# facebookresearch/detectron2

Measured on NVIDIA H100. Metric: Mask R-CNN R50-FPN training hot-path images/sec (custom-op path fwd+bwd, 2 images/GPU), higher is better.
Workload: dtype f32

## Files before the change

detectron2_b200/csrc/deform_conv_tc.cu:

```cuda
#include <algorithm>
#include <cstdlib>

#include "common.cuh"
#include "tc_common.cuh"

using namespace d2b_tc;

namespace {

constexpr int kWorkerWarps = 16;
constexpr int kWorkers = kWorkerWarps * 32;
constexpr int kThreads = kWorkers + 128;
constexpr int kLaunchRegs = (65536 / kThreads) & ~7;
constexpr int kWorkerRegs = 112, kSideRegs = 24;
static_assert(kWorkers * kWorkerRegs + (kThreads - kWorkers) * kSideRegs <= kThreads * kLaunchRegs,
              "register budget exceeds the launch allocation");
constexpr int kMaxBN = 128;
constexpr int kRowsPerHalf = 128 / (2 * kWorkerWarps);
constexpr int kTile = 16384;
constexpr int kMaxSmem = 227 * 1024;
constexpr int kGcolPitch = 132;

struct TC {
  int N, Cin, H, W, Cout, kh, kw, sh, sw, ph, pw, dh, dw, G, DG, Ho, Wo, cpg, opg, cpdg, KK, HoWo;
  int pack, SG, cps, ops, cbs, U;
  int tiles_img;
  int stages_img;
  int MC;
  int nks;
  long long off_bs, mask_bs;
  int mask_sigmoid;
};

struct Epi {
  const float* scale;
  const float* shift;
  int relu;
};

struct K1P { int BN, noct, goct, nkp, ksplit, S, tap_bytes, stage_bytes, red; };
struct K2P { int mper, msplit, tap_bytes; };
struct K3P { int BN, noct, sper, nsplit, S, stage_bytes; };

inline size_t align256(size_t v) { return (v + 255) & ~(size_t)255; }

bool make_tc(const d2b_dcn_params* p, TC& d) {
  if (!p) return false;
  d.N = p->N; d.Cin = p->Cin; d.H = p->H; d.W = p->W; d.Cout = p->Cout; d.kh = p->kh; d.kw = p->kw;
// ... 172 lines not shown
  const float* __restrict__ p = xcb + (uint32_t)(code >> 4) * Cin;
  const float4 z = make_float4(0.f, 0.f, 0.f, 0.f);
  t.v0 = (code & 1) ? __ldg(reinterpret_cast<const float4*>(p)) : z;
  t.v1 = (code & 2) ? __ldg(reinterpret_cast<const float4*>(p + Cin)) : z;
  t.v2 = (code & 4) ? __ldg(reinterpret_cast<const float4*>(p + rs)) : z;
  t.v3 = (code & 8) ? __ldg(reinterpret_cast<const float4*>(p + (rs + Cin))) : z;
}

__device__ __forceinline__ void interp4(const Taps4& t, float w0, float w1, float w2, float w3, float (&v)[4]) {
  const F2 z = f2_pack(0.f, 0.f), p0 = f2_pack(w0, w0), p1 = f2_pack(w1, w1), p2 = f2_pack(w2, w2), p3 = f2_pack(w3, w3);
  F2 a = f2_fma(p0, f2_pack(t.v0.x, t.v0.y), z), b = f2_fma(p0, f2_pack(t.v0.z, t.v0.w), z);
  a = f2_fma(p1, f2_pack(t.v1.x, t.v1.y), a);
  b = f2_fma(p1, f2_pack(t.v1.z, t.v1.w), b);
  a = f2_fma(p2, f2_pack(t.v2.x, t.v2.y), a);
  b = f2_fma(p2, f2_pack(t.v2.z, t.v2.w), b);
  a = f2_fma(p3, f2_pack(t.v3.x, t.v3.y), a);
  b = f2_fma(p3, f2_pack(t.v3.z, t.v3.w), b);
  f2_unpack(a, v[0], v[1]);
  f2_unpack(b, v[2], v[3]);
}

__device__ __forceinline__ void gather_store(const Taps4& t, int4 tap, uint8_t* a_hi, uint8_t* a_lo, uint32_t off,
                                             bool split) {
  const float lh = __int_as_float(tap.y), lw = __int_as_float(tap.z), m = __int_as_float(tap.w);
  const float hh = 1.f - lh, hw = 1.f - lw;
  float v[4];
  interp4(t, hh * hw * m, hh * lw * m, lh * hw * m, lh * lw * m, v);
  uint2 hi, lo;
  split4(v, hi, lo);
  *reinterpret_cast<uint2*>(a_hi + off) = hi;
  if (split) *reinterpret_cast<uint2*>(a_lo + off) = lo;
}

template <int BN, int kTransA, int kSplit>
__device__ __forceinline__ void mma_stage_(float (&acc)[BN / 4], uint32_t a_hi, uint32_t a_lo, uint32_t b_hi, uint32_t b_lo) {
  const int g = (threadIdx.x >> 7);
  const uint32_t ao = kTransA ? (uint32_t)(g & 1) * 8192u : (uint32_t)(g & 1) * 64u * 128u;
  const uint32_t bo = (uint32_t)(g >> 1) * (uint32_t)(BN / 2) * 128u;
  const uint32_t lbo = kTransA ? 8192u : 0u;
  wgmma_fence();
#pragma unroll
  for (int kk = 0; kk < 4; ++kk) {
    const uint32_t ak = ao + (kTransA ? (uint32_t)kk * 2048u : (uint32_t)kk * 32u), bk = bo + (uint32_t)kk * 32u;
    Wgmma<BN / 2, kTransA>::mma(acc, wgmma_desc(a_hi + ak, lbo, 1024), wgmma_desc(b_hi + bk, 0, 1024), 1);
    if (kSplit) {
      Wgmma<BN / 2, kTransA>::mma(acc, wgmma_desc(a_hi + ak, lbo, 1024), wgmma_desc(b_lo + bk, 0, 1024), 1);
      Wgmma<BN / 2, kTransA>::mma(acc, wgmma_desc(a_lo + ak, lbo, 1024), wgmma_desc(b_hi + bk, 0, 1024), 1);
    }
  }
  wgmma_commit();
}
template <int BN, int kTransA>
__device__ __forceinline__ void mma_stage(float (&acc)[BN / 4], uint32_t a_hi, uint32_t a_lo, uint32_t b_hi, uint32_t b_lo,
                                          int split) {
  if (split) mma_stage_<BN, kTransA, 1>(acc, a_hi, a_lo, b_hi, b_lo);
  else mma_stage_<BN, kTransA, 0>(acc, a_hi, a_lo, b_hi, b_lo);
}

template <int BN>
__device__ __forceinline__ int acc_row(int i) {
  const int t = threadIdx.x & 127;
  return (threadIdx.x >> 7 & 1) * 64 + (t >> 5) * 16 + ((t & 31) >> 2) + ((i >> 1) & 1) * 8;
}
template <int BN>
__device__ __forceinline__ int acc_col(int i) {
  return (threadIdx.x >> 8) * (BN / 2) + (i >> 2) * 8 + (threadIdx.x & 3) * 2 + (i & 1);
}

template <int BN>
__device__ __forceinline__ void fwd_epilogue(const float (&acc)[BN / 4], const Epi& ep, const TC& d, const K1P& k,
                                             float* __restrict__ out, int b, int p0, int oc0) {
  const bool add_shift = ep.shift != nullptr && blockIdx.z == 0;
#pragma unroll
  for (int i = 0; i < BN / 4; ++i) {
    const int p = p0 + acc_row<BN>(i);
    if (p >= d.HoWo) continue;
    const int oc = oc0 + acc_col<BN>(i);
    float* dst = out + ((size_t)b * d.Cout + oc) * d.HoWo + p;
    float v = acc[i];
    if (k.red) {
      red_add(dst, v + ((add_shift && !ep.scale && !ep.relu) ? __ldg(ep.shift + oc) : 0.f));
    } else {
      if (ep.scale) v *= __ldg(ep.scale + oc);
      if (ep.shift) v += __ldg(ep.shift + oc);
      if (ep.relu) v = fmaxf(v, 0.f);
      *dst = v;
    }
  }
}

template <int BN>
__global__ void __launch_bounds__(kThreads, 1) dcn_fwd_tc_kernel(const float* __restrict__ xh,
                                                                   const float* __restrict__ offset,
                                                                   const float* __restrict__ mask,
                                                                   const uint8_t* __restrict__ wt, const Epi ep, const TC d,
                                                                   const K1P k, const int split, float* __restrict__ out,
                                                                   uint8_t* __restrict__ cols) {
  extern __shared__ uint8_t smem_raw[];
  uint8_t* smem = smem_raw + ((1024u - (smem_u32(smem_raw) & 1023u)) & 1023u);
  int4* taps = reinterpret_cast<int4*>(smem + k.S * k.stage_bytes);
  uint64_t* bars = reinterpret_cast<uint64_t*>(reinterpret_cast<uint8_t*>(taps) + k.tap_bytes);
  uint64_t* full_bar = bars;
  uint64_t* empty_bar = bars + k.S;

  const int tid = threadIdx.x, warp = tid >> 5, lane = tid & 31;
  const int b = blockIdx.x / d.tiles_img, p0 = (blockIdx.x - b * d.tiles_img) * 128;
  const int sg = blockIdx.y / k.goct, oct = blockIdx.y - sg * k.goct;
  const int kp0 = blockIdx.z * k.nkp, nkp = min(d.KK, kp0 + k.nkp) - kp0;
  const int nt = nkp * d.cbs;
  const int dg0 = (sg * d.cps) / d.cpdg;
// ... 23 lines not shown
    const float* __restrict__ ximg = xh + (size_t)b * d.H * d.W * d.Cin - (size_t)(d.W + 1) * d.Cin;
    const uint32_t ucin = (uint32_t)d.Cin, urs = (uint32_t)(d.W * d.Cin);
    float acc[BN / 4];
#pragma unroll
    for (int i = 0; i < BN / 4; ++i) acc[i] = 0.f;
    int kpl = 0, cb = 0;
    auto stage = [&](int t) {
      const int s = t % k.S;
      const uint32_t par = (uint32_t)((t / k.S) & 1);
      const int cbase = sg * d.cps + cb * 64;
      const int4* __restrict__ tp = taps + ((cbase / d.cpdg - dg0) * nkp + kpl) * 128;
      const float* __restrict__ xc = ximg + cbase + q * 4;
      uint8_t* a_hi = smem + s * k.stage_bytes;
      uint8_t* a_lo = a_hi + kTile;
      mbar_wait(&empty_bar[s], par ^ 1u);
      {
        int4 tap[kRowsPerHalf];
        Taps4 c[kRowsPerHalf];
#pragma unroll
        for (int j = 0; j < kRowsPerHalf; ++j) tap[j] = tp[warp * 2 * kRowsPerHalf + j * 2 + half];
#pragma unroll
        for (int j = 0; j < kRowsPerHalf; ++j) load_corners(xc, ucin, urs, tap[j].x, c[j]);
#pragma unroll
        for (int j = 0; j < kRowsPerHalf; ++j) {
          const uint32_t r = (uint32_t)(warp * 2 * kRowsPerHalf + j * 2 + half);
          gather_store(c[j], tap[j], a_hi, a_lo, swz128(r, (uint32_t)(q >> 1)) + (uint32_t)(q & 1) * 8u, split != 0);
        }
      }
      fence_proxy_async();
      __syncwarp();
      if (lane == 0) mbar_arrive(&full_bar[s]);
      mbar_wait(&full_bar[s], par);
      const uint32_t sa = smem_u32(a_hi), sb = sa + 2 * kTile;
      mma_stage<BN, 0>(acc, sa, sa + kTile, sb, sb + (uint32_t)BN * 128u, split);
      if (++cb == d.cbs) { cb = 0; ++kpl; }
    };
    stage(0);
    for (int t = 1; t < nt; ++t) {
      stage(t);
      wgmma_wait<1>();
      __syncwarp();
      if (lane == 0) mbar_arrive(&empty_bar[(t - 1) % k.S]);
    }
    wgmma_wait<0>();
    fwd_epilogue<BN>(acc, ep, d, k, out, b, p0, sg * d.ops + oct * k.BN);
  } else if (warp == kWorkerWarps) {
    if (lane == 0) {
      const uint32_t bytes = (uint32_t)(split ? 2 : 1) * (uint32_t)k.BN * 128u;
      for (int t = 0; t < nt; ++t) {
        const int s = t % k.S;
        const uint32_t par = (uint32_t)((t / k.S) & 1);
        mbar_wait(&empty_bar[s], par ^ 1u);
        const size_t tile = ((size_t)(sg * k.noct + oct) * d.U + (size_t)kp0 * d.cbs + t);
        mbar_arrive_expect_tx(&full_bar[s], bytes);
        bulk_g2s(smem + s * k.stage_bytes + 2 * kTile, wt + tile * (size_t)(2 * k.BN * 128), bytes, &full_bar[s]);
      }
    }
  } else if (warp == kWorkerWarps + 1) {
    if (saving && lane == 0) {
      const uint32_t tile_bytes = (uint32_t)(split ? 2 : 1) * (uint32_t)kTile;
      for (int t = 0; t < nt; ++t) {
        const int s = t % k.S;
        const uint32_t par = (uint32_t)((t / k.S) & 1);
        mbar_wait(&full_bar[s], par);
        const size_t tile = ((size_t)blockIdx.x * d.SG + sg) * d.U + (size_t)kp0 * d.cbs + t;
        bulk_s2g(cols + tile * tile_bytes, smem + s * k.stage_bytes, tile_bytes);
        bulk_commit();
        bulk_wait_read0();
        mbar_arrive(&empty_bar[s]);
      }
      bulk_wait0();
    }
  }
}

template <int BN>
__global__ void __launch_bounds__(kThreads, 1) dcn_fwd_cols_kernel(const uint8_t* __restrict__ cols,
                                                                   const uint8_t* __restrict__ wt, const Epi ep, const TC d,
                                                                   const K1P k, const int split, float* __restrict__ out) {
  extern __shared__ uint8_t smem_raw[];
  uint8_t* smem = smem_raw + ((1024u - (smem_u32(smem_raw) & 1023u)) & 1023u);
  uint64_t* bars = reinterpret_cast<uint64_t*>(smem + k.S * k.stage_bytes);
  uint64_t* full_bar = bars;
  uint64_t* empty_bar = bars + k.S;

  const int tid = threadIdx.x, warp = tid >> 5, lane = tid & 31;
  const int tile = blockIdx.x / k.goct, oct = 1 + (blockIdx.x - tile * k.goct);
  const int b = tile / d.tiles_img, p0 = (tile - b * d.tiles_img) * 128;
  const int sg = blockIdx.y;
  const int kp0 = blockIdx.z * k.nkp, nkp = min(d.KK, kp0 + k.nkp) - kp0;
  const int nt = nkp * d.cbs;

  if (tid == 0) {
    for (int s = 0; s < k.S; ++s) {
      mbar_init(&full_bar[s], 1);
      mbar_init(&empty_bar[s], kWorkerWarps);
    }
    mbar_init_fence();
  }
  __syncthreads();
  if (warp < kWorkerWarps) reg_alloc<kWorkerRegs>();
  else reg_dealloc<kSideRegs>();

  if (warp < kWorkerWarps) {
    float acc[BN / 4];
#pragma unroll
    for (int i = 0; i < BN / 4; ++i) acc[i] = 0.f;
    auto issue = [&](int t) {
      const int s = t % k.S;
      mbar_wait(&full_bar[s], (uint32_t)((t / k.S) & 1));
      const uint32_t sa = smem_u32(smem + s * k.stage_bytes), sb = sa + 2 * kTile;
      mma_stage<BN, 0>(acc, sa, sa + kTile, sb, sb + (uint32_t)BN * 128u, split);
    };
    issue(0);
    for (int t = 1; t < nt; ++t) {
      issue(t);
      wgmma_wait<1>();
      __syncwarp();
      if (lane == 0) mbar_arrive(&empty_bar[(t - 1) % k.S]);
    }
    wgmma_wait<0>();
    fwd_epilogue<BN>(acc, ep, d, k, out, b, p0, sg * d.ops + oct * k.BN);
  } else if (warp == kWorkerWarps) {
    if (lane == 0) {
      const uint32_t parts = split ? 2u : 1u;
      const uint32_t abytes = parts * (uint32_t)kTile;
      const size_t u0 = (size_t)kp0 * d.cbs;
      const uint8_t* asrc = cols + (((size_t)tile * d.SG + sg) * d.U + u0) * abytes;
      const uint8_t* bsrc = wt + ((size_t)(sg * k.noct + oct) * d.U + u0) * (size_t)(2 * BN * 128);
      int s = 0;
      uint32_t par = 1u;
      for (int t = nt; t > 0; --t, asrc += abytes, bsrc += 2 * BN * 128) {
        mbar_wait(&empty_bar[s], par);
        mbar_arrive_expect_tx(&full_bar[s], abytes / 128u * (128u + BN));
        bulk_g2s(smem + s * k.stage_bytes, asrc, abytes, &full_bar[s]);
        bulk_g2s(smem + s * k.stage_bytes + 2 * kTile, bsrc, abytes / 128u * BN, &full_bar[s]);
        if (++s == k.S) {
          s = 0;
          par ^= 1u;
        }
      }
    }
  }
}

__global__ void __launch_bounds__(kThreads, 1) dcn_bwd_data_tc_kernel(const float* __restrict__ xh,
                                                                      const float* __restrict__ offset,
                                                                      const float* __restrict__ mask,
                                                                      const uint8_t* __restrict__ gt,
                                                                      const uint8_t* __restrict__ wt, const TC d,
                                                                      const K2P k, const int split,
                                                                      float* __restrict__ gxh, float* __restrict__ goff,
                                                                      float* __restrict__ gmask) {
  extern __shared__ uint8_t smem_raw[];
  uint8_t* smem = smem_raw + ((1024u - (smem_u32(smem_raw) & 1023u)) & 1023u);
  constexpr int kStage = 4 * kTile;
// ... 71 lines not shown
      float v = (b1 ? u1 : u0) + __shfl_xor_sync(0xffffffffu, b1 ? u0 : u1, 1);
      {
        const int j = q >> 2, which = q & 3;
        const int row = warp * 2 * R + j * 2 + half;
        const int p = p0 + row;
        if (which < 3 && p < d.HoWo) {
          if (which < 2) {
            if (goff) red_add(goff + (size_t)b * d.off_bs + ((size_t)cur_dg * 2 * d.KK + 2 * cur_kp + which) * d.HoWo + p, v);
          } else if (gmask) {
            if (d.mask_sigmoid) {
              const float m = __int_as_float(taps[((cur_dg - dg0) * nkp + (cur_kp - kp0)) * 128 + row].w);
              v *= m * (1.f - m);
            }
            red_add(gmask + (size_t)b * d.mask_bs + ((size_t)cur_dg * d.KK + cur_kp) * d.HoWo + p, v);
          }
        }
      }
#pragma unroll
      for (int j = 0; j < R; ++j) sh[j] = sw[j] = sm[j] = 0.f;
    };

    for (int ml = 0; ml < nm; ++ml) {
      const int buf = ml & 1;
      const int m = m0 + ml;
      const int nu = (2 * m + 1 < d.U) ? 2 : 1;
      {
        float acc[32];
#pragma unroll
        for (int i = 0; i < 32; ++i) acc[i] = 0.f;
        for (int ks = 0; ks < d.nks; ++ks) {
          const int c = ml * d.nks + ks, s = c & 1;
          mbar_wait(&full_bar[s], (uint32_t)((c >> 1) & 1));
          const uint32_t sa = smem_u32(smem + s * kStage);
          mma_stage<128, 0>(acc, sa, sa + kTile, sa + 2 * kTile, sa + 3 * kTile, split);
          wgmma_wait<0>();
          __syncwarp();
          if (lane == 0) mbar_arrive(&empty_bar[s]);
        }
#pragma unroll
        for (int i = 0; i < 32; i += 2)
          *reinterpret_cast<float2*>(gcol + acc_row<128>(i) * kGcolPitch + acc_col<128>(i)) = make_float2(acc[i], acc[i + 1]);
      }
      named_bar_sync(1, kWorkers);
      for (int ul = 0; ul < nu; ++ul) {
        const int u = 2 * m + ul;
        const int kp = u / d.cbs, cb = u - kp * d.cbs;
        const int cbase = sg * d.cps + cb * 64;
        const int dg = cbase / d.cpdg;
        if (kp != cur_kp || dg != cur_dg) {
          flush();
          cur_kp = kp;
          cur_dg = dg;
        }
        const int4* __restrict__ tp = taps + ((dg - dg0) * nkp + (kp - kp0)) * 128;
        const float* __restrict__ xc = ximg + cbase + q * 4;
        float* __restrict__ gc = gimg + cbase + q * 4;
        constexpr int kB2 = 2;
#pragma unroll
        for (int it = 0; it < R / kB2; ++it) {
          int4 tap[kB2];
          Taps4 c[kB2];
#pragma unroll
          for (int e = 0; e < kB2; ++e) tap[e] = tp[warp * 2 * R + (it * kB2 + e) * 2 + half];
#pragma unroll
          for (int e = 0; e < kB2; ++e) load_corners(xc, ucin, urs, tap[e].x, c[e]);
#pragma unroll
          for (int e = 0; e < kB2; ++e) {
            if ((tap[e].x & 15) == 0) continue;
            const int j = it * kB2 + e;
            const int row = warp * 2 * R + j * 2 + half;
            const float4 g4 = *reinterpret_cast<const float4*>(gcol + row * kGcolPitch + ul * 64 + q * 4);
            const float lh = __int_as_float(tap[e].y), lw = __int_as_float(tap[e].z), mk = __int_as_float(tap[e].w);
            const float hh = 1.f - lh, hw = 1.f - lw;
            const float w0 = hh * hw, w1 = hh * lw, w2 = lh * hw, w3 = lh * lw;
// ... 30 lines not shown
              float* gp = gc + (uint32_t)(tap[e].x >> 4) * ucin;
              red_add_v4_if(tap[e].x & 1, gp, f2_mul(GM[0], W0), f2_mul(GM[1], W0));
              red_add_v4_if(tap[e].x & 2, gp + ucin, f2_mul(GM[0], W1), f2_mul(GM[1], W1));
              red_add_v4_if(tap[e].x & 4, gp + urs, f2_mul(GM[0], W2), f2_mul(GM[1], W2));
              red_add_v4_if(tap[e].x & 8, gp + (urs + ucin), f2_mul(GM[0], W3), f2_mul(GM[1], W3));
            }
          }
        }
      }
      named_bar_sync(1, kWorkers);
    }
    flush();
  } else if (warp == kWorkerWarps) {
    if (lane == 0) {
      const uint32_t half_bytes = (uint32_t)(split ? 2 : 1) * (uint32_t)kTile;
      int c = 0;
      for (int ml = 0; ml < nm; ++ml) {
        const int m = m0 + ml;
        for (int ks = 0; ks < d.nks; ++ks, ++c) {
          const int s = c & 1;
          const uint32_t par = (uint32_t)((c >> 1) & 1);
          mbar_wait(&empty_bar[s], par ^ 1u);
          mbar_arrive_expect_tx(&full_bar[s], 2 * half_bytes);
          const size_t atile = (((size_t)b * d.tiles_img + pt) * d.SG + sg) * d.nks + ks;
          const size_t btile = ((size_t)sg * d.MC + m) * d.nks + ks;
          bulk_g2s(smem + s * kStage, gt + atile * (size_t)(2 * kTile), half_bytes, &full_bar[s]);
          bulk_g2s(smem + s * kStage + 2 * kTile, wt + btile * (size_t)(2 * kTile), half_bytes, &full_bar[s]);
        }
      }
    }
  }
}

template <int BN>
__device__ __forceinline__ void gw_tile_store(const float (&acc)[BN / 4], float* __restrict__ tile, int pitch) {
#pragma unroll
  for (int i = 0; i < BN / 4; i += 2) red_add_v2(tile + (size_t)acc_row<BN>(i) * pitch + acc_col<BN>(i), acc[i], acc[i + 1]);
}

__global__ void dcn_gw_reduce_kernel(const float* __restrict__ part, const TC d, float* __restrict__ gw) {
  const long long total = (long long)d.SG * d.U * 64 * d.ops;
  const long long idx = (long long)blockIdx.x * blockDim.x + threadIdx.x;
  if (idx >= total) return;
  const int ocl = (int)(idx % d.ops);
  const long long r = idx / d.ops;
  const int rowu = (int)(r % ((long long)d.U * 64)), sg = (int)(r / ((long long)d.U * 64));
  const int u = rowu >> 6, ch = rowu & 63;
  const int kp = u / d.cbs, cb = u - kp * d.cbs;
  const int ec = sg * d.cps + cb * 64 + ch, egrp = ec / d.cpg, ecin = ec - egrp * d.cpg;
  const int oc = sg * d.ops + ocl;
  if (oc / d.opg != egrp) return;
  gw[((size_t)oc * d.cpg + ecin) * d.KK + kp] = __ldg(part + ((size_t)sg * d.MC * 128 + rowu) * d.ops + ocl);
}

constexpr int kRedOc = 16, kRedCh = 16;
__global__ void __launch_bounds__(256) dcn_gw_reduce_tile_kernel(const float* __restrict__ part, const TC d,
                                                                  float* __restrict__ gw) {
  __shared__ float tile[9 * kRedCh][kRedOc + 1];
  const int per_sg = d.cps / kRedCh;
  const int sg = blockIdx.x / per_sg, c0 = (blockIdx.x - sg * per_sg) * kRedCh;
  const int cb = c0 >> 6, ch0 = c0 & 63;
  const int ocl0 = blockIdx.y * kRedOc;
  const int tid = threadIdx.x;
  {
    const int j = tid & (kRedOc - 1), r0 = tid / kRedOc;
    for (int row = r0; row < d.KK * kRedCh; row += 256 / kRedOc) {
      const int kp = row / kRedCh, ch = row - kp * kRedCh;
      tile[row][j] = __ldg(part + ((size_t)sg * d.MC * 128 + (size_t)(kp * d.cbs + cb) * 64 + ch0 + ch) * d.ops + ocl0 + j);
    }
  }
// ... 75 lines not shown
      const bool have_next = i + 1 < ns;
      TapRaw raw = {0.f, 0.f, 1.f};
      if (have_next) {
        stage_of(i + 1, bn, pbn);
        if (tl_ok) raw = tap_loads(d, offset, mask, bn, tl_dg, tl_kp, pbn + warp * PX + tl_j);
      }
      const float* __restrict__ xc = xh + ((size_t)b * d.H * d.W - (size_t)(d.W + 1)) * d.Cin + cbase + q * 4;
      const uint32_t ucin = (uint32_t)d.Cin, urs = (uint32_t)(d.W * d.Cin);
      uint8_t* a_hi = smem + s * k.stage_bytes + half * 8192;
      uint8_t* a_lo = a_hi + kTile;
      const int4* cur = my_taps + (i & 1) * (2 * PX) + half * PX;
      mbar_wait(&empty_bar[s], par ^ 1u);
      {
        int4 tap[PX];
        Taps4 c[PX];
#pragma unroll
        for (int j = 0; j < PX; ++j) tap[j] = cur[j];
#pragma unroll
        for (int j = 0; j < PX; ++j) load_corners(xc, ucin, urs, tap[j].x, c[j]);
#pragma unroll
        for (int j = 0; j < PX; ++j) {
          const uint32_t r = (uint32_t)(warp * PX + j);
          gather_store(c[j], tap[j], a_hi, a_lo, swz128(r, (uint32_t)(q >> 1)) + (uint32_t)(q & 1) * 8u, split != 0);
        }
      }
      if (have_next && lane < 2 * PX)
        my_taps[((i + 1) & 1) * (2 * PX) + lane] =
            tl_ok ? tap_finish(d, raw, mask != nullptr, tl_kp, pbn + warp * PX + tl_j) : make_int4(0, 0, 0, 0);
      fence_proxy_async();
      __syncwarp();
      if (lane == 0) mbar_arrive(&full_bar[s]);
      mbar_wait(&full_bar[s], par);
      const uint32_t sa = smem_u32(smem + s * k.stage_bytes), sb = sa + 2 * kTile;
      mma_stage<BN, 1>(acc, sa, sa + kTile, sb, sb + (uint32_t)BN * 128u, split);
    };
    stage(0);
    for (int i = 1; i < ns; ++i) {
      stage(i);
      wgmma_wait<1>();
      __syncwarp();
      if (lane == 0) mbar_arrive(&empty_bar[(i - 1) % k.S]);
    }
    wgmma_wait<0>();
    gw_tile_store<BN>(acc, gw + ((size_t)sg * d.MC * 128 + (size_t)mb * 128) * d.ops + (size_t)oct * k.BN, d.ops);
  } else if (warp == kWorkerWarps) {
    if (lane == 0) {
      const uint32_t bytes = (uint32_t)(split ? 2 : 1) * (uint32_t)k.BN * 128u;
      for (int i = 0; i < ns; ++i) {
        const int s = i % k.S;
        const uint32_t par = (uint32_t)((i / k.S) & 1);
        mbar_wait(&empty_bar[s], par ^ 1u);
        mbar_arrive_expect_tx(&full_bar[s], bytes);
        const size_t tile = ((size_t)(gs0 + i) * d.SG + sg) * k.noct + oct;
        bulk_g2s(smem + s * k.stage_bytes + 2 * kTile, gt + tile * (size_t)(2 * k.BN * 128), bytes, &full_bar[s]);
      }
    }
  }
}

template <int BN>
__global__ void __launch_bounds__(kThreads, 1) dcn_bwd_weight_cols_kernel(const uint8_t* __restrict__ cols,
                                                                          const uint8_t* __restrict__ gt, const TC d,
                                                                          const K3P k, const int S, const int split,
                                                                          float* __restrict__ gw) {
  extern __shared__ uint8_t smem_raw[];
  uint8_t* smem = smem_raw + ((1024u - (smem_u32(smem_raw) & 1023u)) & 1023u);
  uint64_t* bars = reinterpret_cast<uint64_t*>(smem + S * k.stage_bytes);
  uint64_t* full_bar = bars;
  uint64_t* empty_bar = bars + S;

  const int tid = threadIdx.x, warp = tid >> 5, lane = tid & 31;
  const int mb = blockIdx.y;
  const int sg = blockIdx.x / k.noct, oct = blockIdx.x - sg * k.noct;
  const int total = d.N * d.stages_img;
  const int gs0 = blockIdx.z * k.sper, gs1 = min(total, gs0 + k.sper), ns = gs1 - gs0;
  const int nu = (2 * mb + 1 < d.U) ? 2 : 1;

  if (tid == 0) {
    for (int s = 0; s < S; ++s) {
      mbar_init(&full_bar[s], 1);
      mbar_init(&empty_bar[s], kWorkerWarps);
    }
    mbar_init_fence();
  }
  if (nu == 1 && tid < kWorkers) {
    for (int s = 0; s < S; ++s)
      for (int i = tid; i < 2 * 512; i += kWorkers) {
        const int part = i >> 9, w = i & 511;
        reinterpret_cast<uint4*>(smem + s * k.stage_bytes + part * kTile + 8192)[w] = make_uint4(0, 0, 0, 0);
      }
    fence_proxy_async();
  }
  __syncthreads();
  if (warp < kWorkerWarps) reg_alloc<kWorkerRegs>();
  else reg_dealloc<kSideRegs>();

  if (warp < kWorkerWarps) {
    float acc[BN / 4];
#pragma unroll
    for (int i = 0; i < BN / 4; ++i) acc[i] = 0.f;
    auto issue = [&](int i) {
      const int s = i % S;
      mbar_wait(&full_bar[s], (uint32_t)((i / S) & 1));
      const uint32_t sa = smem_u32(smem + s * k.stage_bytes), sb = sa + 2 * kTile;
      mma_stage<BN, 1>(acc, sa, sa + kTile, sb, sb + (uint32_t)BN * 128u, split);
    };
    issue(0);
    for (int i = 1; i < ns; ++i) {
      issue(i);
      wgmma_wait<1>();
      __syncwarp();
      if (lane == 0) mbar_arrive(&empty_bar[(i - 1) % S]);
    }
    wgmma_wait<0>();
    gw_tile_store<BN>(acc, gw + ((size_t)sg * d.MC * 128 + (size_t)mb * 128) * d.ops + (size_t)oct * k.BN, d.ops);
  } else if (warp == kWorkerWarps) {
    if (lane == 0) {
      const uint32_t parts = split ? 2u : 1u;
      const uint32_t tile_bytes = parts * (uint32_t)kTile;
      const uint32_t gbytes = parts * (uint32_t)k.BN * 128u;
      for (int i = 0; i < ns; ++i) {
        const int s = i % S;
        const uint32_t par = (uint32_t)((i / S) & 1);
        const int gs = gs0 + i;
        const int b = gs / d.stages_img, st = gs - b * d.stages_img;
        mbar_wait(&empty_bar[s], par ^ 1u);
        mbar_arrive_expect_tx(&full_bar[s], (uint32_t)nu * parts * 8192u + gbytes);
        uint8_t* stage = smem + s * k.stage_bytes;
        const uint8_t* src =
            cols + ((((size_t)b * d.tiles_img + (st >> 1)) * d.SG + sg) * d.U + 2 * mb) * tile_bytes + (size_t)(st & 1) * 8192;
        for (int ul = 0; ul < nu; ++ul)
          for (uint32_t part = 0; part < parts; ++part)
            bulk_g2s(stage + part * kTile + ul * 8192, src + (size_t)ul * tile_bytes + (size_t)part * kTile, 8192u, &full_bar[s]);
        const size_t tile = ((size_t)gs * d.SG + sg) * k.noct + oct;
        bulk_g2s(stage + 2 * kTile, gt + tile * (size_t)(2 * k.BN * 128), gbytes, &full_bar[s]);
      }
    }
  }
}

__device__ __forceinline__ void split8(const float (&v)[8], uint4& hi, uint4& lo) {
  split2(v[0], v[1], hi.x, lo.x);
  split2(v[2], v[3], hi.y, lo.y);
  split2(v[4], v[5], hi.z, lo.z);
  split2(v[6], v[7], hi.w, lo.w);
}

__device__ __forceinline__ float w_elem(const float* __restrict__ w, const TC& d, int oc, int c, int kp) {
  const int g = c / d.cpg;
// ... 243 lines not shown
  K1P kc;
  bool colfed = false;
  if (cols && k.noct > 1) {
    K1P k1;
    if (plan_k1(d, k1, true) && plan_k1c(d, k1, kc)) {
      k = k1;
      colfed = true;
    }
  }
  if (k.red) D2B_CUDA(cudaMemsetAsync(out, 0, sizeof(float) * (size_t)d.N * d.Cout * d.HoWo, stream));
  const int smem_bytes = k.S * k.stage_bytes + k.tap_bytes + 1024 + 128;
  const int split = precision == 1 ? 1 : 0;
  const Epi ep = {scale, shift, relu};
  dim3 grid(d.N * d.tiles_img, d.SG * k.goct, k.ksplit);
#define D2B_LAUNCH_K1(BN)                                                                                              \
  {                                                                                                                    \
    D2B_ALLOW_BIG_SMEM(dcn_fwd_tc_kernel<BN>);                                                                         \
    dcn_fwd_tc_kernel<BN><<<grid, kThreads, smem_bytes, stream>>>(xh, offset, mask, wt, ep, d, k, split, out,        \
                                                                    reinterpret_cast<uint8_t*>(cols));                 \
  }
  if (k.BN == 16) D2B_LAUNCH_K1(16)
  else if (k.BN == 32) D2B_LAUNCH_K1(32)
  else if (k.BN == 64) D2B_LAUNCH_K1(64)
  else D2B_LAUNCH_K1(128)
#undef D2B_LAUNCH_K1
  D2B_CHECK_LAUNCH();
  if (colfed) {
    const int smem_c = kc.S * kc.stage_bytes + 1024 + 128;
    dim3 grid_c(d.N * d.tiles_img * kc.goct, d.SG, kc.ksplit);
    const uint8_t* cl = reinterpret_cast<const uint8_t*>(cols);
#define D2B_LAUNCH_K1C(BN)                                                                                             \
  {                                                                                                                    \
    D2B_ALLOW_BIG_SMEM(dcn_fwd_cols_kernel<BN>);                                                                       \
    dcn_fwd_cols_kernel<BN><<<grid_c, kThreads, smem_c, stream>>>(cl, wt, ep, d, kc, split, out);                      \
  }
    if (kc.BN == 16) D2B_LAUNCH_K1C(16)
    else if (kc.BN == 32) D2B_LAUNCH_K1C(32)
    else if (kc.BN == 64) D2B_LAUNCH_K1C(64)
    else D2B_LAUNCH_K1C(128)
#undef D2B_LAUNCH_K1C
    D2B_CHECK_LAUNCH();
  }
  if (k.red && (scale || relu)) {
    const long long total = (long long)d.N * d.Cout * d.HoWo;
    dcn_epilogue_kernel<<<d2b_cdiv(total, 256), 256, 0, stream>>>(out, total, d.Cout, d.HoWo, ep);
    D2B_CHECK_LAUNCH();
  }
  return D2B_OK;
}

size_t d2b_deform_conv_tc_bwd_workspace(const d2b_dcn_params* p, int x_nhwc, int need_data, int need_weight) {
  TC d;
  K2P k2;
  K3P k3;
  if (!make_tc(p, d) || !plan_k2(d, k2) || !plan_k3(d, k3)) return 0;
  size_t b = 0;
  const size_t xbytes = align256(sizeof(float) * (size_t)d.N * d.H * d.W * d.Cin);
  if (!x_nhwc) b += xbytes;
  if (need_data && !x_nhwc) b += xbytes;
  if (need_data) {
    b += align256((size_t)d.N * d.tiles_img * d.SG * d.nks * 2 * kTile);
    b += align256((size_t)d.SG * d.MC * d.nks * 2 * kTile);
  }
  if (need_weight) {
    b += align256((size_t)d.N * d.stages_img * d.SG * k3.noct * 2 * k3.BN * 128);
    b += align256(sizeof(float) * (size_t)d.SG * d.MC * 128 * d.ops);
  }
// ... 70 lines not shown
        grad_out, y_saved, ep, d, gt_px, gt_oc, k3.BN, k3.noct);
    D2B_CHECK_LAUNCH();
    {
      const long long total = (long long)d.SG * d.MC * d.nks * 128 * 8;
      dcn_wtile_bwd_kernel<<<d2b_cdiv(total, 256), 256, 0, stream>>>(weight, d, wt);
      D2B_CHECK_LAUNCH();
    }
    const int smem_bytes = 2 * 4 * kTile + 128 * kGcolPitch * 4 + k2.tap_bytes + 1024 + 128;
    D2B_ALLOW_BIG_SMEM(dcn_bwd_data_tc_kernel);
    dim3 grid(d.N * d.tiles_img, d.SG, k2.msplit);
    dcn_bwd_data_tc_kernel<<<grid, kThreads, smem_bytes, stream>>>(xh, offset, mask, gt_px, wt, d, k2, split, gxh, grad_offset,
                                                                  mask ? grad_mask : nullptr);
    D2B_CHECK_LAUNCH();
    if (grad_x && !x_nhwc) {
      dim3 g2(d2b_cdiv(d.H * d.W, 64), d2b_cdiv(d.Cin, 32), d.N);
      nhwc_to_nchw_kernel<<<g2, 256, 0, stream>>>(gxh, d.Cin, d.H * d.W, grad_x);
      D2B_CHECK_LAUNCH();
    }
  }
  if (need_weight) {
    if (!need_data) {
      const long long total = (long long)d.N * d.stages_img * d.SG * k3.noct * k3.BN * 8;
      dcn_gout_oc_tiles_kernel<<<d2b_cdiv(total, 256), 256, 0, stream>>>(grad_out, y_saved, ep, d, k3.BN, k3.noct, gt_oc);
      D2B_CHECK_LAUNCH();
    }
    dim3 grid(d.SG * k3.noct, d.MC, k3.nsplit);
    if (cols) {
      const int S = std::min(6, (kMaxSmem - 2048) / k3.stage_bytes);
      const int smem_bytes = S * k3.stage_bytes + 1024 + 128;
      const uint8_t* cl = reinterpret_cast<const uint8_t*>(cols);
#define D2B_LAUNCH_K3C(BN)                                                                                             \
  {                                                                                                                      \
    D2B_ALLOW_BIG_SMEM(dcn_bwd_weight_cols_kernel<BN>);                                                                \
    dcn_bwd_weight_cols_kernel<BN><<<grid, kThreads, smem_bytes, stream>>>(cl, gt_oc, d, k3, S, split, gw_part);       \
  }
      if (k3.BN == 64) D2B_LAUNCH_K3C(64)
      else D2B_LAUNCH_K3C(128)
#undef D2B_LAUNCH_K3C
    } else {
      const int smem_bytes = k3.S * k3.stage_bytes + 4096 + 1024 + 128;
#define D2B_LAUNCH_K3(BN)                                                                                              \
  {                                                                                                                      \
    D2B_ALLOW_BIG_SMEM(dcn_bwd_weight_tc_kernel<BN>);                                                                  \
    dcn_bwd_weight_tc_kernel<BN><<<grid, kThreads, smem_bytes, stream>>>(xh, offset, mask, gt_oc, d, k3, split, gw_part); \
  }
      if (k3.BN == 64) D2B_LAUNCH_K3(64)
      else D2B_LAUNCH_K3(128)
#undef D2B_LAUNCH_K3
    }
    D2B_CHECK_LAUNCH();
    {
      if (d.KK <= 9) {
        dcn_gw_reduce_tile_kernel<<<dim3(d.SG * (d.cps / kRedCh), d.ops / kRedOc), 256, 0, stream>>>(gw_part, d, grad_weight);
      } else {
        const long long total = (long long)d.SG * d.U * 64 * d.ops;
        dcn_gw_reduce_kernel<<<d2b_cdiv(total, 256), 256, 0, stream>>>(gw_part, d, grad_weight);
      }
      D2B_CHECK_LAUNCH();
    }
  }
  return D2B_OK;
}
```

Measured before the change: 284.2.

## Use two consumer warpgroups with wider WGMMA tiles in cols-fed deform-conv kernels

The column-fed forward and weight-gradient deform-conv kernels now run two consumer warpgroups instead of four, each issuing WGMMA over the full BN width with doubled accumulators and a larger register allocation (232 per consumer thread). The MMA stage helper is parameterised by warpgroup count so the gather kernels keep the four-warpgroup split. The aim is to cut per-instruction overhead and thread count where no gather work is needed, at the cost of higher register pressure and fewer warps to hide latency. Descriptors are also hoisted and reused across split passes.

```diff
diff --git a/detectron2_b200/csrc/deform_conv_tc.cu b/detectron2_b200/csrc/deform_conv_tc.cu
--- a/detectron2_b200/csrc/deform_conv_tc.cu
+++ b/detectron2_b200/csrc/deform_conv_tc.cu
@@ -14,6 +14,13 @@
 constexpr int kLaunchRegs = (65536 / kThreads) & ~7;
 constexpr int kWorkerRegs = 112, kSideRegs = 24;
 static_assert(kWorkers * kWorkerRegs + (kThreads - kWorkers) * kSideRegs <= kThreads * kLaunchRegs,
+              "register budget exceeds the launch allocation");
+constexpr int kColsConsumers = 256;
+constexpr int kColsThreads = kColsConsumers + 128;
+constexpr int kColsLaunchRegs = (65536 / kColsThreads) & ~7;
+constexpr int kColsConsumerRegs = 232, kColsProducerRegs = 40;
+static_assert(kColsConsumers * kColsConsumerRegs + (kColsThreads - kColsConsumers) * kColsProducerRegs <=
+                  kColsThreads * kColsLaunchRegs,
               "register budget exceeds the launch allocation");
 constexpr int kMaxBN = 128;
 constexpr int kRowsPerHalf = 128 / (2 * kWorkerWarps);
@@ -252,50 +259,53 @@
   if (split) *reinterpret_cast<uint2*>(a_lo + off) = lo;
 }
 
-template <int BN, int kTransA, int kSplit>
-__device__ __forceinline__ void mma_stage_(float (&acc)[BN / 4], uint32_t a_hi, uint32_t a_lo, uint32_t b_hi, uint32_t b_lo) {
+template <int BN, int kWG, int kTransA, int kSplit>
+__device__ __forceinline__ void mma_stage_(float (&acc)[BN / kWG], uint32_t a_hi, uint32_t a_lo, uint32_t b_hi, uint32_t b_lo) {
+  static_assert(kWG == 2 || kWG == 4, "two or four warpgroups per tile");
+  constexpr int WN = 2 * BN / kWG;
   const int g = (threadIdx.x >> 7);
   const uint32_t ao = kTransA ? (uint32_t)(g & 1) * 8192u : (uint32_t)(g & 1) * 64u * 128u;
-  const uint32_t bo = (uint32_t)(g >> 1) * (uint32_t)(BN / 2) * 128u;
+  const uint32_t bo = kWG == 4 ? (uint32_t)(g >> 1) * (uint32_t)WN * 128u : 0u;
   const uint32_t lbo = kTransA ? 8192u : 0u;
   wgmma_fence();
 #pragma unroll
   for (int kk = 0; kk < 4; ++kk) {
     const uint32_t ak = ao + (kTransA ? (uint32_t)kk * 2048u : (uint32_t)kk * 32u), bk = bo + (uint32_t)kk * 32u;
-    Wgmma<BN / 2, kTransA>::mma(acc, wgmma_desc(a_hi + ak, lbo, 1024), wgmma_desc(b_hi + bk, 0, 1024), 1);
+    const uint64_t dah = wgmma_desc(a_hi + ak, lbo, 1024), dbh = wgmma_desc(b_hi + bk, 0, 1024);
+    Wgmma<WN, kTransA>::mma(acc, dah, dbh, 1);
     if (kSplit) {
-      Wgmma<BN / 2, kTransA>::mma(acc, wgmma_desc(a_hi + ak, lbo, 1024), wgmma_desc(b_lo + bk, 0, 1024), 1);
-      Wgmma<BN / 2, kTransA>::mma(acc, wgmma_desc(a_lo + ak, lbo, 1024), wgmma_desc(b_hi + bk, 0, 1024), 1);
+      Wgmma<WN, kTransA>::mma(acc, dah, wgmma_desc(b_lo + bk, 0, 1024), 1);
+      Wgmma<WN, kTransA>::mma(acc, wgmma_desc(a_lo + ak, lbo, 1024), dbh, 1);
     }
   }
   wgmma_commit();
 }
-template <int BN, int kTransA>
-__device__ __forceinline__ void mma_stage(float (&acc)[BN / 4], uint32_t a_hi, uint32_t a_lo, uint32_t b_hi, uint32_t b_lo,
+template <int BN, int kWG, int kTransA>
+__device__ __forceinline__ void mma_stage(float (&acc)[BN / kWG], uint32_t a_hi, uint32_t a_lo, uint32_t b_hi, uint32_t b_lo,
                                           int split) {
-  if (split) mma_stage_<BN, kTransA, 1>(acc, a_hi, a_lo, b_hi, b_lo);
-  else mma_stage_<BN, kTransA, 0>(acc, a_hi, a_lo, b_hi, b_lo);
-}
-
-template <int BN>
+  if (split) mma_stage_<BN, kWG, kTransA, 1>(acc, a_hi, a_lo, b_hi, b_lo);
+  else mma_stage_<BN, kWG, kTransA, 0>(acc, a_hi, a_lo, b_hi, b_lo);
+}
+
 __device__ __forceinline__ int acc_row(int i) {
   const int t = threadIdx.x & 127;
   return (threadIdx.x >> 7 & 1) * 64 + (t >> 5) * 16 + ((t & 31) >> 2) + ((i >> 1) & 1) * 8;
 }
-template <int BN>
+template <int BN, int kWG>
 __device__ __forceinline__ int acc_col(int i) {
-  return (threadIdx.x >> 8) * (BN / 2) + (i >> 2) * 8 + (threadIdx.x & 3) * 2 + (i & 1);
-}
-
-template <int BN>
-__device__ __forceinline__ void fwd_epilogue(const float (&acc)[BN / 4], const Epi& ep, const TC& d, const K1P& k,
+  const int c0 = kWG == 4 ? (int)(threadIdx.x >> 8) * (BN / 2) : 0;
+  return c0 + (i >> 2) * 8 + (threadIdx.x & 3) * 2 + (i & 1);
+}
+
+template <int BN, int kWG>
+__device__ __forceinline__ void fwd_epilogue(const float (&acc)[BN / kWG], const Epi& ep, const TC& d, const K1P& k,
                                              float* __restrict__ out, int b, int p0, int oc0) {
   const bool add_shift = ep.shift != nullptr && blockIdx.z == 0;
 #pragma unroll
-  for (int i = 0; i < BN / 4; ++i) {
-    const int p = p0 + acc_row<BN>(i);
+  for (int i = 0; i < BN / kWG; ++i) {
+    const int p = p0 + acc_row(i);
     if (p >= d.HoWo) continue;
-    const int oc = oc0 + acc_col<BN>(i);
+    const int oc = oc0 + acc_col<BN, kWG>(i);
     float* dst = out + ((size_t)b * d.Cout + oc) * d.HoWo + p;
     float v = acc[i];
     if (k.red) {
@@ -385,7 +395,7 @@
       if (lane == 0) mbar_arrive(&full_bar[s]);
       mbar_wait(&full_bar[s], par);
       const uint32_t sa = smem_u32(a_hi), sb = sa + 2 * kTile;
-      mma_stage<BN, 0>(acc, sa, sa + kTile, sb, sb + (uint32_t)BN * 128u, split);
+      mma_stage<BN, 4, 0>(acc, sa, sa + kTile, sb, sb + (uint32_t)BN * 128u, split);
       if (++cb == d.cbs) { cb = 0; ++kpl; }
     };
     stage(0);
@@ -396,7 +406,7 @@
       if (lane == 0) mbar_arrive(&empty_bar[(t - 1) % k.S]);
     }
     wgmma_wait<0>();
-    fwd_epilogue<BN>(acc, ep, d, k, out, b, p0, sg * d.ops + oct * k.BN);
+    fwd_epilogue<BN, 4>(acc, ep, d, k, out, b, p0, sg * d.ops + oct * k.BN);
   } else if (warp == kWorkerWarps) {
     if (lane == 0) {
       const uint32_t bytes = (uint32_t)(split ? 2 : 1) * (uint32_t)k.BN * 128u;
@@ -428,9 +438,11 @@
 }
 
 template <int BN>
-__global__ void __launch_bounds__(kThreads, 1) dcn_fwd_cols_kernel(const uint8_t* __restrict__ cols,
-                                                                   const uint8_t* __restrict__ wt, const Epi ep, const TC d,
-                                                                   const K1P k, const int split, float* __restrict__ out) {
+__global__ void __launch_bounds__(kColsThreads, 1) dcn_fwd_cols_kernel(const uint8_t* __restrict__ cols,
+                                                                       const uint8_t* __restrict__ wt, const Epi ep,
+                                                                       const TC d, const K1P k, const int split,
+                                                                       float* __restrict__ out) {
+  constexpr int kConsumerWarps = kColsConsumers / 32;
   extern __shared__ uint8_t smem_raw[];
   uint8_t* smem = smem_raw + ((1024u - (smem_u32(smem_raw) & 1023u)) & 1023u);
   uint64_t* bars = reinterpret_cast<uint64_t*>(smem + k.S * k.stage_bytes);
@@ -447,23 +459,23 @@
   if (tid == 0) {
     for (int s = 0; s < k.S; ++s) {
       mbar_init(&full_bar[s], 1);
-      mbar_init(&empty_bar[s], kWorkerWarps);
+      mbar_init(&empty_bar[s], kConsumerWarps);
     }
     mbar_init_fence();
   }
   __syncthreads();
-  if (warp < kWorkerWarps) reg_alloc<kWorkerRegs>();
-  else reg_dealloc<kSideRegs>();
-
-  if (warp < kWorkerWarps) {
-    float acc[BN / 4];
-#pragma unroll
-    for (int i = 0; i < BN / 4; ++i) acc[i] = 0.f;
+  if (warp < kConsumerWarps) reg_alloc<kColsConsumerRegs>();
+  else reg_dealloc<kColsProducerRegs>();
+
+  if (warp < kConsumerWarps) {
+    float acc[BN / 2];
+#pragma unroll
+    for (int i = 0; i < BN / 2; ++i) acc[i] = 0.f;
     auto issue = [&](int t) {
       const int s = t % k.S;
       mbar_wait(&full_bar[s], (uint32_t)((t / k.S) & 1));
       const uint32_t sa = smem_u32(smem + s * k.stage_bytes), sb = sa + 2 * kTile;
-      mma_stage<BN, 0>(acc, sa, sa + kTile, sb, sb + (uint32_t)BN * 128u, split);
+      mma_stage<BN, 2, 0>(acc, sa, sa + kTile, sb, sb + (uint32_t)BN * 128u, split);
     };
     issue(0);
     for (int t = 1; t < nt; ++t) {
@@ -473,8 +485,8 @@
       if (lane == 0) mbar_arrive(&empty_bar[(t - 1) % k.S]);
     }
     wgmma_wait<0>();
-    fwd_epilogue<BN>(acc, ep, d, k, out, b, p0, sg * d.ops + oct * k.BN);
-  } else if (warp == kWorkerWarps) {
+    fwd_epilogue<BN, 2>(acc, ep, d, k, out, b, p0, sg * d.ops + oct * k.BN);
+  } else if (warp == kConsumerWarps) {
     if (lane == 0) {
       const uint32_t parts = split ? 2u : 1u;
       const uint32_t abytes = parts * (uint32_t)kTile;
@@ -612,14 +624,14 @@
           const int c = ml * d.nks + ks, s = c & 1;
           mbar_wait(&full_bar[s], (uint32_t)((c >> 1) & 1));
           const uint32_t sa = smem_u32(smem + s * kStage);
-          mma_stage<128, 0>(acc, sa, sa + kTile, sa + 2 * kTile, sa + 3 * kTile, split);
+          mma_stage<128, 4, 0>(acc, sa, sa + kTile, sa + 2 * kTile, sa + 3 * kTile, split);
           wgmma_wait<0>();
           __syncwarp();
           if (lane == 0) mbar_arrive(&empty_bar[s]);
         }
 #pragma unroll
         for (int i = 0; i < 32; i += 2)
-          *reinterpret_cast<float2*>(gcol + acc_row<128>(i) * kGcolPitch + acc_col<128>(i)) = make_float2(acc[i], acc[i + 1]);
+          *reinterpret_cast<float2*>(gcol + acc_row(i) * kGcolPitch + acc_col<128, 4>(i)) = make_float2(acc[i], acc[i + 1]);
       }
       named_bar_sync(1, kWorkers);
       for (int ul = 0; ul < nu; ++ul) {
@@ -716,10 +728,11 @@
   }
 }
 
-template <int BN>
-__device__ __forceinline__ void gw_tile_store(const float (&acc)[BN / 4], float* __restrict__ tile, int pitch) {
-#pragma unroll
-  for (int i = 0; i < BN / 4; i += 2) red_add_v2(tile + (size_t)acc_row<BN>(i) * pitch + acc_col<BN>(i), acc[i], acc[i + 1]);
+template <int BN, int kWG>
+__device__ __forceinline__ void gw_tile_store(const float (&acc)[BN / kWG], float* __restrict__ tile, int pitch) {
+#pragma unroll
+  for (int i = 0; i < BN / kWG; i += 2)
+    red_add_v2(tile + (size_t)acc_row(i) * pitch + acc_col<BN, kWG>(i), acc[i], acc[i + 1]);
 }
 
 __global__ void dcn_gw_reduce_kernel(const float* __restrict__ part, const TC d, float* __restrict__ gw) {
@@ -861,7 +874,7 @@
       if (lane == 0) mbar_arrive(&full_bar[s]);
       mbar_wait(&full_bar[s], par);
       const uint32_t sa = smem_u32(smem + s * k.stage_bytes), sb = sa + 2 * kTile;
-      mma_stage<BN, 1>(acc, sa, sa + kTile, sb, sb + (uint32_t)BN * 128u, split);
+      mma_stage<BN, 4, 1>(acc, sa, sa + kTile, sb, sb + (uint32_t)BN * 128u, split);
     };
     stage(0);
     for (int i = 1; i < ns; ++i) {
@@ -871,7 +884,7 @@
       if (lane == 0) mbar_arrive(&empty_bar[(i - 1) % k.S]);
     }
     wgmma_wait<0>();
-    gw_tile_store<BN>(acc, gw + ((size_t)sg * d.MC * 128 + (size_t)mb * 128) * d.ops + (size_t)oct * k.BN, d.ops);
+    gw_tile_store<BN, 4>(acc, gw + ((size_t)sg * d.MC * 128 + (size_t)mb * 128) * d.ops + (size_t)oct * k.BN, d.ops);
   } else if (warp == kWorkerWarps) {
     if (lane == 0) {
       const uint32_t bytes = (uint32_t)(split ? 2 : 1) * (uint32_t)k.BN * 128u;
@@ -888,10 +901,11 @@
 }
 
 template <int BN>
-__global__ void __launch_bounds__(kThreads, 1) dcn_bwd_weight_cols_kernel(const uint8_t* __restrict__ cols,
-                                                                          const uint8_t* __restrict__ gt, const TC d,
-                                                                          const K3P k, const int S, const int split,
-                                                                          float* __restrict__ gw) {
+__global__ void __launch_bounds__(kColsThreads, 1) dcn_bwd_weight_cols_kernel(const uint8_t* __restrict__ cols,
+                                                                              const uint8_t* __restrict__ gt, const TC d,
+                                                                              const K3P k, const int S, const int split,
+                                                                              float* __restrict__ gw) {
+  constexpr int kConsumerWarps = kColsConsumers / 32;
   extern __shared__ uint8_t smem_raw[];
   uint8_t* smem = smem_raw + ((1024u - (smem_u32(smem_raw) & 1023u)) & 1023u);
   uint64_t* bars = reinterpret_cast<uint64_t*>(smem + S * k.stage_bytes);
@@ -908,31 +922,31 @@
   if (tid == 0) {
     for (int s = 0; s < S; ++s) {
       mbar_init(&full_bar[s], 1);
-      mbar_init(&empty_bar[s], kWorkerWarps);
+      mbar_init(&empty_bar[s], kConsumerWarps);
     }
     mbar_init_fence();
   }
-  if (nu == 1 && tid < kWorkers) {
+  if (nu == 1 && tid < kColsConsumers) {
     for (int s = 0; s < S; ++s)
-      for (int i = tid; i < 2 * 512; i += kWorkers) {
+      for (int i = tid; i < 2 * 512; i += kColsConsumers) {
         const int part = i >> 9, w = i & 511;
         reinterpret_cast<uint4*>(smem + s * k.stage_bytes + part * kTile + 8192)[w] = make_uint4(0, 0, 0, 0);
       }
     fence_proxy_async();
   }
   __syncthreads();
-  if (warp < kWorkerWarps) reg_alloc<kWorkerRegs>();
-  else reg_dealloc<kSideRegs>();
-
-  if (warp < kWorkerWarps) {
-    float acc[BN / 4];
-#pragma unroll
-    for (int i = 0; i < BN / 4; ++i) acc[i] = 0.f;
+  if (warp < kConsumerWarps) reg_alloc<kColsConsumerRegs>();
+  else reg_dealloc<kColsProducerRegs>();
+
+  if (warp < kConsumerWarps) {
+    float acc[BN / 2];
+#pragma unroll
+    for (int i = 0; i < BN / 2; ++i) acc[i] = 0.f;
     auto issue = [&](int i) {
       const int s = i % S;
       mbar_wait(&full_bar[s], (uint32_t)((i / S) & 1));
       const uint32_t sa = smem_u32(smem + s * k.stage_bytes), sb = sa + 2 * kTile;
-      mma_stage<BN, 1>(acc, sa, sa + kTile, sb, sb + (uint32_t)BN * 128u, split);
+      mma_stage<BN, 2, 1>(acc, sa, sa + kTile, sb, sb + (uint32_t)BN * 128u, split);
     };
     issue(0);
     for (int i = 1; i < ns; ++i) {
@@ -942,8 +956,8 @@
       if (lane == 0) mbar_arrive(&empty_bar[(i - 1) % S]);
     }
     wgmma_wait<0>();
-    gw_tile_store<BN>(acc, gw + ((size_t)sg * d.MC * 128 + (size_t)mb * 128) * d.ops + (size_t)oct * k.BN, d.ops);
-  } else if (warp == kWorkerWarps) {
+    gw_tile_store<BN, 2>(acc, gw + ((size_t)sg * d.MC * 128 + (size_t)mb * 128) * d.ops + (size_t)oct * k.BN, d.ops);
+  } else if (warp == kConsumerWarps) {
     if (lane == 0) {
       const uint32_t parts = split ? 2u : 1u;
       const uint32_t tile_bytes = parts * (uint32_t)kTile;
@@ -1253,7 +1267,7 @@
 #define D2B_LAUNCH_K1C(BN)                                                                                             \
   {                                                                                                                    \
     D2B_ALLOW_BIG_SMEM(dcn_fwd_cols_kernel<BN>);                                                                       \
-    dcn_fwd_cols_kernel<BN><<<grid_c, kThreads, smem_c, stream>>>(cl, wt, ep, d, kc, split, out);                      \
+    dcn_fwd_cols_kernel<BN><<<grid_c, kColsThreads, smem_c, stream>>>(cl, wt, ep, d, kc, split, out);                      \
   }
     if (kc.BN == 16) D2B_LAUNCH_K1C(16)
     else if (kc.BN == 32) D2B_LAUNCH_K1C(32)
@@ -1390,7 +1404,7 @@
 #define D2B_LAUNCH_K3C(BN)                                                                                             \
   {                                                                                                                      \
     D2B_ALLOW_BIG_SMEM(dcn_bwd_weight_cols_kernel<BN>);                                                                \
-    dcn_bwd_weight_cols_kernel<BN><<<grid, kThreads, smem_bytes, stream>>>(cl, gt_oc, d, k3, S, split, gw_part);       \
+    dcn_bwd_weight_cols_kernel<BN><<<grid, kColsThreads, smem_bytes, stream>>>(cl, gt_oc, d, k3, S, split, gw_part);       \
   }
       if (k3.BN == 64) D2B_LAUNCH_K3C(64)
       else D2B_LAUNCH_K3C(128)
```

After: 288.8 (median of 6 runs). 1.02x the previous value.
